# cyberfabric/cyberfabric-core

Measured on NVIDIA H100. Metric: prompt_bytes_per_sec_bpe_encode, higher is better.
Workload: dtype u32

## Files before the change

cyberfabric-core_b200/csrc/bpe_kernels.cuh:

```cuda
#pragma once
#include <stdint.h>

#include "pretok.cuh"
#include "pretok_fsm.h"
#include "pretok_sync.cuh"
#include "specials.h"
#include "tables.h"
#include "tma.cuh"

namespace cfbpe {

#ifdef CUSIM_EMULATOR
#define CFBPE_DYN_SMEM(name) uint32_t* const name = reinterpret_cast<uint32_t*>(cusim::dyn_smem())
#else
#define CFBPE_DYN_SMEM(name) extern __shared__ __align__(16) uint32_t name[]
#endif

constexpr uint32_t kMaxVocabs = 8;
#ifdef CUSIM_EMULATOR
inline unsigned long long* dbg_counters() { static unsigned long long c[16]; return c; }
#define CFBPE_DBG_COUNT(i) (++dbg_counters()[i])
#else
#define CFBPE_DBG_COUNT(i) ((void)0)
#endif
// ... 283 lines not shown
                                const uint64_t w0 = w << 5;
                                uint32_t m = pat_bits << off;
                                if (e < w0 + 32u) m &= (1u << static_cast<uint32_t>(e - w0)) - 1u;
                                if (m) atomicOr(&piece_bits[w], m);
                                off = off % md + adv; if (off >= md) off -= md;
                            }
                        }
                    }
                    state = S_D1 + static_cast<uint32_t>((d - 1u + (e - pos)) % md);
                    pos = e; prevx = X_N; nlet = 0; npun = 0;
                }
            }
#if defined(CFBPE_TILE_CLOCK) && !defined(CUSIM_EMULATOR)
            rs_bulk += clock64() - rs_b0;
#endif
        }
    }
    if (!kFix) {
        or_bits(piece_bits, cs >> 5, static_cast<uint32_t>(mine));
        or_bits(piece_bits, (cs >> 5) + 1, static_cast<uint32_t>(mine >> 32));
    }
    if (bad) atomicOr(&status->bad_utf8, 1u);
}

__global__ void __launch_bounds__(256)
pretok_split_kernel(BatchView b, VocabSet vs, UcTables uc, uint32_t* __restrict__ piece_bits, DeviceStatus* status, SplitFix* fix_list, uint32_t fix_cap) {
    __shared__ uint16_t s_fsm[kNumPatterns * kPretokTableSize];
    __shared__ uint8_t s_ascii[128];
    for (uint32_t i = threadIdx.x; i < kNumPatterns * kPretokTableSize; i += blockDim.x) s_fsm[i] = uc.fsm[i];
    if (threadIdx.x < 128) s_ascii[threadIdx.x] = uc.ascii_x[threadIdx.x];
    __syncthreads();
    const uint64_t chunk = static_cast<uint64_t>(blockIdx.x) * blockDim.x + threadIdx.x;
    const uint64_t cs = chunk * kSplitChunk;
    if (cs >= b.total_bytes) return;
    const uint64_t ce = (cs + kSplitChunk < b.total_bytes) ? cs + kSplitChunk : b.total_bytes;
    split_thread<0>(b, vs, uc, s_fsm, s_ascii, piece_bits, status, fix_list, fix_cap, cs, ce, 0, 0);
}

__global__ void __launch_bounds__(256)
pretok_fixup_kernel(BatchView b, VocabSet vs, UcTables uc, uint32_t* __restrict__ piece_bits, DeviceStatus* status, const SplitFix* fix_list, uint32_t fix_cap) {
    __shared__ uint16_t s_fsm[kNumPatterns * kPretokTableSize];
    __shared__ uint8_t s_ascii[128];
    const uint32_t n = status->fix_n < fix_cap ? status->fix_n : fix_cap;
    if (blockIdx.x * blockDim.x >= n) return;
    for (uint32_t i = threadIdx.x; i < kNumPatterns * kPretokTableSize; i += blockDim.x) s_fsm[i] = uc.fsm[i];
    if (threadIdx.x < 128) s_ascii[threadIdx.x] = uc.ascii_x[threadIdx.x];
    __syncthreads();
    for (uint32_t i = blockIdx.x * blockDim.x + threadIdx.x; i < n; i += gridDim.x * blockDim.x) {
        const SplitFix f = fix_list[i];
        split_thread<1>(b, vs, uc, s_fsm, s_ascii, piece_bits, status, nullptr, 0, 0, f.ce, f.pos, 0xFFFFFFFFu);
    }
}


constexpr uint32_t kFull = 0xFFFFFFFFu;

__device__ __forceinline__ uint32_t lanemask_lt(uint32_t lane) { return (1u << lane) - 1u; }

__device__ __forceinline__ uint64_t load_bits33(const uint32_t* __restrict__ bits, uint64_t n_words, uint64_t ws) {
    const uint64_t w = ws >> 5;
    const uint32_t sh = static_cast<uint32_t>(ws & 31);
    const uint64_t lo = bits[w];
    const uint64_t hi = (w + 1 < n_words) ? bits[w + 1] : 0;
    const uint64_t v = (lo | (hi << 32)) >> sh;
    return v & 0x1FFFFFFFFull;
}

__device__ __forceinline__ uint64_t next_set_bit(const uint32_t* __restrict__ bits, uint64_t from, uint64_t limit) {
    if (from >= limit) return limit;
    uint64_t w = from >> 5;
    uint32_t cur = bits[w] & (kFull << (from & 31));
    const uint64_t wl = (limit + 31) >> 5;
    while (!cur) {
        if (++w >= wl) return limit;
        cur = bits[w];
    }
    const uint64_t p = (w << 5) + (__ffs(cur) - 1);
    return p < limit ? p : limit;
}


constexpr uint32_t kPieceRange = 512;
constexpr uint32_t kPieceWarps = 4;

__device__ __forceinline__ void load16(const uint8_t* __restrict__ p, uint32_t& w0, uint32_t& w1, uint32_t& w2, uint32_t& w3) {
    const uintptr_t addr = reinterpret_cast<uintptr_t>(p);
    const uint32_t* q = reinterpret_cast<const uint32_t*>(addr & ~static_cast<uintptr_t>(3));
    const uint32_t sh = static_cast<uint32_t>(addr & 3) * 8;
    const uint32_t a = q[0], bq = q[1], c = q[2], d = q[3];
    if (sh == 0) { w0 = a; w1 = bq; w2 = c; w3 = d; }
    else {
        const uint32_t e = q[4];
        w0 = __funnelshift_r(a, bq, sh); w1 = __funnelshift_r(bq, c, sh); w2 = __funnelshift_r(c, d, sh); w3 = __funnelshift_r(d, e, sh);
    }
}

__device__ __forceinline__ uint32_t whole_piece_lookup(const TablesView& T, const uint8_t* __restrict__ p, uint32_t len) {
    if (len > T.max_token_len) return kNone;
    uint32_t w0, w1, w2, w3;
    load16(p, w0, w1, w2, w3);
    uint64_t k0 = static_cast<uint64_t>(w0) | (static_cast<uint64_t>(w1) << 32);
    uint32_t k1 = w2;
    if (len < 8) k0 &= (1ull << (8 * len)) - 1ull;
    if (len <= 8) k1 = 0; else if (len < 12) k1 &= (1u << (8 * (len - 8))) - 1u;
    if (len <= kShortMaxLen) return short_lookup(T, k0, k1, len);
    return long_lookup(T, long_hash(k0, k1, load_le32(p + len - 4), len), p, len);
}

__device__ __forceinline__ uint32_t merge_piece_in_lane(const TablesView& T, const uint8_t* __restrict__ text, uint64_t pos, uint32_t len,
                                                        uint32_t* sid, uint32_t* srk, uint32_t* __restrict__ tok_bits) {
    const uint8_t* __restrict__ p = text + pos;
    uint32_t w[8];
    load16(p, w[0], w[1], w[2], w[3]);
    if (len > 16) load16(p + 16, w[4], w[5], w[6], w[7]); else { w[4] = w[5] = w[6] = w[7] = 0; }
    auto byte_at = [&](uint32_t k) -> uint32_t {
        const uint32_t lo4 = (k & 4u) ? ((k & 8u) ? ((k & 16u) ? w[7] : w[3]) : ((k & 16u) ? w[5] : w[1]))
                                       : ((k & 8u) ? ((k & 16u) ? w[6] : w[2]) : ((k & 16u) ? w[4] : w[0]));
        return (lo4 >> (8u * (k & 3u))) & 0xFFu;
    };
    for (uint32_t k0 = 0; k0 < len; k0 += 4) {
        uint32_t bv[5], idv[4], rkv[4];
#pragma unroll
        for (uint32_t t = 0; t < 5; ++t) bv[t] = (k0 + t < len) ? byte_at(k0 + t) : 0u;
#pragma unroll
        for (uint32_t t = 0; t < 4; ++t) {
            idv[t] = (k0 + t < len) ? T.byte2id[bv[t]] : 0u;
            rkv[t] = (k0 + t + 1 < len) ? T.bytepair[(bv[t] << 8) | bv[t + 1]] : kNone;
        }
#pragma unroll
        for (uint32_t t = 0; t < 4; ++t) if (k0 + t < len) { sid[(k0 + t) * 32] = idv[t]; srk[(k0 + t) * 32] = rkv[t] == kNone ? kNone : ((rkv[t] << 5) | (k0 + t)); }
    }
    uint32_t alive = (len >= 32) ? kFull : ((1u << len) - 1u);
    for (;;) {
        uint32_t bkey = kNone;
        for (uint32_t bits = alive; bits; bits &= bits - 1) {
            const uint32_t k = static_cast<uint32_t>(__ffs(bits)) - 1u;
            const uint32_t r = srk[k * 32];
            bkey = r < bkey ? r : bkey;
        }
        if (bkey == kNone) break;
        const uint32_t best = bkey >> 5, bi = bkey & 31u;
        const uint32_t above = alive & ~((2u << bi) - 1u);
        const uint32_t nb = static_cast<uint32_t>(__ffs(above)) - 1u;
        alive &= ~(1u << nb);
        sid[bi * 32] = best;
        const uint32_t above2 = alive & ~((2u << bi) - 1u);
        const uint32_t below = alive & ((1u << bi) - 1u);
        const bool wr = above2 != 0, wl = below != 0;
        const uint32_t nn = wr ? static_cast<uint32_t>(__ffs(above2)) - 1u : 0u;
        const uint32_t pv = wl ? 31u - static_cast<uint32_t>(__clz(below)) : 0u;
        uint32_t nr, nl;
        pair_lookup2(T, best, wr ? sid[nn * 32] : 0u, wr, wl ? sid[pv * 32] : 0u, best, wl, nr, nl);
        srk[bi * 32] = nr == kNone ? kNone : ((nr << 5) | bi);
        if (wl) srk[pv * 32] = nl == kNone ? kNone : ((nl << 5) | pv);
    }
    const uint64_t mask = static_cast<uint64_t>(alive) << (pos & 31);
    atomicOr(&tok_bits[pos >> 5], static_cast<uint32_t>(mask));
    if (mask >> 32) atomicOr(&tok_bits[(pos >> 5) + 1], static_cast<uint32_t>(mask >> 32));
    return alive;
}

__device__ __forceinline__ uint32_t kth_set_bit(uint32_t mask, uint32_t k) {
    for (uint32_t i = 0; i < k; ++i) mask &= mask - 1;
    return __ffs(mask) - 1;
}

constexpr uint32_t kPieceMulti = 0x80000000u;
constexpr uint32_t kPieceLong = 0xFFFFFFFEu;
constexpr uint32_t kPieceTileBytes = kPieceWarps * kPieceRange;
static_assert(kPieceTileBytes == 64 * 32, "K3 derives a word's piece tile as word >> 6");
struct DenseIds {
    uint32_t* by_piece;
    uint32_t* extras;
    uint32_t extras_cap;
    uint32_t* tile_pieces;
    uint64_t* piece_base;
};

__global__ void __launch_bounds__(kPieceWarps * 32)
long_scan_kernel(BatchView b, const uint32_t* __restrict__ piece_bits, LongPiece* __restrict__ long_list, uint32_t long_cap,
                 DeviceStatus* status, uint32_t* __restrict__ tile_pieces) {
    const uint32_t lane = threadIdx.x & 31, wic = threadIdx.x >> 5;
    const uint64_t warp = static_cast<uint64_t>(blockIdx.x) * kPieceWarps + wic;
    const uint64_t r0 = warp * kPieceRange;
    const uint64_t r1 = (r0 + kPieceRange < b.total_bytes) ? r0 + kPieceRange : b.total_bytes;
    const bool multi = b.vocab_ids != nullptr;
    const uint64_t base = r0 + 16ull * lane;
    const uint32_t my = (base < b.total_bytes) ? ((piece_bits[base >> 5] >> (16u * (lane & 1u))) & 0xFFFFu) : 0u;
    uint32_t v = my ? (16u * lane + static_cast<uint32_t>(__ffs(my)) - 1u) : 0xFFFFu;
#pragma unroll
    for (uint32_t d = 1; d < 32; d <<= 1) { const uint32_t o = __shfl_down_sync(kFull, v, d); if (lane + d < 32 && o < v) v = o; }
    uint32_t nf_rel = __shfl_down_sync(kFull, v, 1);
    if (lane == 31) nf_rel = 0xFFFFu;
    const bool any_open = __any_sync(kFull, my != 0 && nf_rel == 0xFFFFu);
    uint64_t beyond = b.total_bytes;
    if (any_open) beyond = next_set_bit(piece_bits, r1, b.total_bytes);
    const uint64_t nf = (nf_rel == 0xFFFFu) ? beyond : r0 + nf_rel;
    __shared__ uint32_t s_n[2], s_at[2], s_pieces;
    __shared__ unsigned long long s_bytes;
    if (threadIdx.x < 2) s_n[threadIdx.x] = 0;
    if (threadIdx.x == 0) { s_bytes = 0; s_pieces = 0; }
    __syncthreads();
    const uint32_t np = __reduce_add_sync(kFull, static_cast<uint32_t>(__popc(my)));
    if (lane == 0 && np) atomicAdd(&s_pieces, np);
    bool is_long = false, big = false;
    uint32_t k = 0, pv = 0;
    uint64_t pos = 0;
    if (my && r0 < b.total_bytes) {
        pos = base + (31u - static_cast<uint32_t>(__clz(my)));
        if (nf - pos > 32) {
            is_long = true;
            big = (nf - pos) > kBigPiece;
            pv = multi ? b.vocab_ids[find_prompt(b.offsets, b.n_prompts, pos)] : 0u;
            k = atomicAdd(&s_n[big ? 1 : 0], 1u);
            atomicAdd(&s_bytes, static_cast<unsigned long long>(nf - pos));
        }
    }
    __syncthreads();
    if (threadIdx.x < 2 && s_n[threadIdx.x]) s_at[threadIdx.x] = atomicAdd(threadIdx.x ? &status->n_big : &status->n_long, s_n[threadIdx.x]);
    if (threadIdx.x == 2 && s_bytes) atomicAdd(&status->long_bytes, s_bytes);
    if (threadIdx.x == 3) tile_pieces[blockIdx.x] = s_pieces;
    __syncthreads();
    if (is_long) {
        const uint32_t idx = s_at[big ? 1 : 0] + k;
        if (idx < long_cap) { LongPiece lp; lp.start = pos; lp.end = nf; lp.vocab = pv; lp.pad = 0; long_list[big ? long_cap - 1 - idx : idx] = lp; }
        else atomicOr(&status->long_overflow, 1u);
    }
}

constexpr uint32_t kLookupWarps = 4;
static_assert(kLookupWarps == kPieceWarps, "K2a's CTA is the 2 KiB tile K2s counted");
__global__ void __launch_bounds__(kLookupWarps * 32)
bpe_lookup_kernel(BatchView b, VocabSet vs, const uint32_t* __restrict__ piece_bits, DenseIds dn, MissLists ml, DeviceStatus* status) {
    __shared__ uint16_t s_pos[kLookupWarps][kPieceRange + 2];
    __shared__ uint64_t s_miss0[kLookupWarps * kPieceRange / 13 + 8];
    __shared__ uint64_t s_miss1[kLookupWarps * kPieceRange / 7 + 8];
    __shared__ uint64_t s_miss2[kLookupWarps * kPieceRange / 2 + 8];
    __shared__ uint32_t s_cnt[3], s_base[3], s_nw[kLookupWarps];
    const uint32_t lane = threadIdx.x & 31, wic = threadIdx.x >> 5;
    if (threadIdx.x < 3) s_cnt[threadIdx.x] = 0;
    const uint64_t warp = static_cast<uint64_t>(blockIdx.x) * kLookupWarps + wic;
    const uint64_t r0 = warp * kPieceRange;
    const uint8_t* __restrict__ text = b.bytes;
    const bool multi = b.vocab_ids != nullptr;
    const bool in_range = r0 < b.total_bytes;
    const uint64_t r1 = (r0 + kPieceRange < b.total_bytes) ? r0 + kPieceRange : b.total_bytes;
    uint32_t n_w = 0;
    if (in_range) {
        const uint64_t base = r0 + 16ull * lane;
        const uint32_t my = (base < b.total_bytes) ? ((piece_bits[base >> 5] >> (16u * (lane & 1u))) & 0xFFFFu) : 0u;
        const uint32_t cnt = __popc(my);
        uint32_t incl = cnt;
#pragma unroll
        for (uint32_t d = 1; d < 32; d <<= 1) { const uint32_t o = __shfl_up_sync(kFull, incl, d); if (lane >= d) incl += o; }
        n_w = __shfl_sync(kFull, incl, 31);
        uint32_t slot = incl - cnt;
        for (uint32_t bits = my; bits; bits &= bits - 1) s_pos[wic][slot++] = static_cast<uint16_t>(16u * lane + static_cast<uint32_t>(__ffs(bits)) - 1u);
    }
    if (lane == 0) s_nw[wic] = n_w;
    __syncthreads();
    if (in_range) {
        uint64_t rank0 = dn.piece_base[blockIdx.x];
        for (uint32_t w = 0; w < wic; ++w) rank0 += s_nw[w];
        uint64_t beyond = b.total_bytes;
        if (n_w) beyond = next_set_bit(piece_bits, r1, b.total_bytes);
        TablesView T = vs.v[0];
        uint32_t vid = 0;
        for (uint32_t i = lane; i < n_w; i += 32) {
            const uint32_t off = s_pos[wic][i];
            const uint64_t pos = r0 + off;
            const uint64_t end = (i + 1 < n_w) ? r0 + s_pos[wic][i + 1] : beyond;
            if (end - pos > 32) { dn.by_piece[rank0 + i] = kPieceLong; continue; }
            const uint32_t len = static_cast<uint32_t>(end - pos);
            if (multi) {
                const uint32_t pv = b.vocab_ids[find_prompt(b.offsets, b.n_prompts, pos)];
                if (pv != vid) { vid = pv; T = vs.v[vid]; }
            }
            const uint32_t tok = (len == 1) ? T.byte2id[text[pos]] : whole_piece_lookup(T, text + pos, len);
            if (tok != kNone) {
                dn.by_piece[rank0 + i] = tok;
            } else {
                const uint32_t c = len >= 13 ? 0u : (len >= 7 ? 1u : 2u);
                const uint32_t k = atomicAdd(&s_cnt[c], 1u);
                (c == 0 ? s_miss0 : (c == 1 ? s_miss1 : s_miss2))[k] = pos | ((rank0 + i) << 32);
            }
        }
    }
    __syncthreads();
    if (threadIdx.x < 3) {
        const uint32_t n = s_cnt[threadIdx.x];
        uint32_t g = n ? atomicAdd(&status->miss_n[threadIdx.x], n) : 0u;
        if (n && g + n > ml.cap[threadIdx.x]) { atomicOr(&status->miss_overflow, 1u); g = 0xFFFFFFFFu; }
        s_base[threadIdx.x] = g;
    }
    __syncthreads();
#pragma unroll
    for (uint32_t c = 0; c < 3; ++c) {
        const uint32_t n = s_cnt[c], g = s_base[c];
        if (g == 0xFFFFFFFFu) continue;
        const uint64_t* src = c == 0 ? s_miss0 : (c == 1 ? s_miss1 : s_miss2);
        for (uint32_t i = threadIdx.x; i < n; i += blockDim.x) ml.list[c][g + i] = src[i];
    }
}

__global__ void __launch_bounds__(kPieceWarps * 32)
bpe_merge_kernel(BatchView b, VocabSet vs, const uint32_t* __restrict__ piece_bits, DenseIds dn,
                 uint32_t* __restrict__ tok_bits, MissLists ml, DeviceStatus* status) {
    __shared__ uint32_t s_id[kPieceWarps][32][32];
    __shared__ uint32_t s_rk[kPieceWarps][32][32];
    const uint32_t lane = threadIdx.x & 31, wic = threadIdx.x >> 5;
    const uint8_t* __restrict__ text = b.bytes;
    const bool multi = b.vocab_ids != nullptr;
    uint32_t* sid = &s_id[wic][0][lane];
    uint32_t* srk = &s_rk[wic][0][lane];
    if (status->miss_overflow) return;
    TablesView T = vs.v[0];
    uint32_t vid = 0;
#pragma unroll 1
    for (uint32_t c = 0; c < 3; ++c) {
        const uint32_t n = status->miss_n[c];
        const uint64_t* __restrict__ list = ml.list[c];
        for (;;) {
            uint32_t t0 = 0;
            if (lane == 0) t0 = atomicAdd(&status->miss_next[c], 32u);
            t0 = __shfl_sync(kFull, t0, 0);
            if (t0 >= n) break;
            const uint32_t i = t0 + lane;
            uint32_t alive = 0, rank = 0;
            if (i < n) {
                const uint64_t e = list[i];
                const uint64_t pos = e & 0xFFFFFFFFull;
                rank = static_cast<uint32_t>(e >> 32);
                const uint64_t end = next_set_bit(piece_bits, pos + 1, b.total_bytes);
                if (multi) {
                    const uint32_t pv = b.vocab_ids[find_prompt(b.offsets, b.n_prompts, pos)];
                    if (pv != vid) { vid = pv; T = vs.v[vid]; }
                }
                alive = merge_piece_in_lane(T, text, pos, static_cast<uint32_t>(end - pos), sid, srk, tok_bits);
            }
            const uint32_t cnt = __popc(alive);
            uint32_t incl = cnt;
#pragma unroll
            for (uint32_t d = 1; d < 32; d <<= 1) { const uint32_t o = __shfl_up_sync(kFull, incl, d); if (lane >= d) incl += o; }
            const uint32_t total = __shfl_sync(kFull, incl, 31);
            uint32_t base = 0;
            if (lane == 0 && total) base = atomicAdd(&status->extra_n, total);
            base = __shfl_sync(kFull, base, 0);
            if (cnt) {
                uint32_t slot = base + incl - cnt;
                if (slot + cnt <= dn.extras_cap) {
                    dn.by_piece[rank] = kPieceMulti | slot;
                    for (uint32_t bits = alive; bits; bits &= bits - 1) dn.extras[slot++] = sid[(static_cast<uint32_t>(__ffs(bits)) - 1u) * 32];
                } else atomicOr(&status->miss_overflow, 1u);
            }
            __syncwarp();
        }
    }
}

struct LongScratch {
    uint32_t* rank;
    uint32_t* aux0;
    uint32_t* aux1;
};

__device__ __forceinline__ uint32_t warp_min_u32(uint32_t v) {
#pragma unroll
    for (uint32_t d = 16; d; d >>= 1) { const uint32_t o = __shfl_xor_sync(kFull, v, d); v = o < v ? o : v; }
    return v;
}

__device__ __forceinline__ bool select_chunk(uint32_t r, uint32_t rmin, uint32_t lane, uint32_t& carry, uint32_t& sel_ballot) {
    const bool cand = (r == rmin);
    const uint32_t C = __ballot_sync(kFull, cand);
    const uint32_t z = ~C & lanemask_lt(lane);
    const uint32_t s = z ? (32u - __clz(z)) : 0u;
    const uint32_t cnt = lane - s + (s == 0 ? carry : 0u);
    const bool sel = cand && !(cnt & 1u);
    sel_ballot = __ballot_sync(kFull, sel);
    const uint32_t nz = ~C;
    carry = nz ? static_cast<uint32_t>(__clz(nz)) : (carry + 32u);
    return sel;
}

// ... 1030 lines not shown
```

cyberfabric-core_b200/csrc/pipeline.cuh:

```cuda
#pragma once
#include "../../include/cfbpe.h"
#include "bpe_kernels.cuh"

namespace cfbpe {

struct Workspace {
    uint32_t* piece_bits;
    uint32_t* tok_bits;
    uint32_t* ids_by_pos;
    LongScratch lscratch;
    LongPiece* long_list;
    uint32_t long_cap;
    uint32_t* tile_counts;
    uint64_t* tile_base;
    DeviceStatus* status;
    MissLists miss;
    SplitFix* fix_list;
    uint32_t fix_cap;
    DenseIds dense;
    uint32_t* pstart_bits;
    uint32_t* block_prompt;
};

enum WsKind : uint32_t {
// ... 32 lines not shown

inline uint64_t miss_list_words(uint64_t max_bytes, uint32_t c, uint32_t max_chunks) {
    return workspace_alloc(max_bytes, max_chunks).n[kWsMiss0 + c];
}

template <typename F>
inline void for_each_ws_buffer(Workspace& w, F&& f) {
    f(w.piece_bits, kWsFlagWords); f(w.tok_bits, kWsFlagWords); f(w.pstart_bits, kWsFlagWords);
    f(w.ids_by_pos, kWsPerByte); f(w.lscratch.rank, kWsPerByte); f(w.lscratch.aux0, kWsPerByte); f(w.lscratch.aux1, kWsPerByte);
    f(w.dense.by_piece, kWsPerByte); f(w.dense.extras, kWsPerByte);
    f(w.long_list, kWsLongList);
    f(w.tile_counts, kWsScanTiles); f(w.tile_base, kWsScanTiles);
    f(w.miss.list[0], kWsMiss0); f(w.miss.list[1], kWsMiss1); f(w.miss.list[2], kWsMiss2);
    f(w.fix_list, kWsFixList);
    f(w.dense.tile_pieces, kWsPieceTiles); f(w.dense.piece_base, kWsPieceTiles);
    f(w.block_prompt, kWsBlockPrompt);
}

inline void set_workspace_caps(Workspace& w, const WsSizes& s) {
    w.long_cap = static_cast<uint32_t>(s.n[kWsLongList]);
    w.fix_cap = static_cast<uint32_t>(s.n[kWsFixList]);
    w.dense.extras_cap = static_cast<uint32_t>(s.n[kWsPerByte]);
    for (uint32_t c = 0; c < 3; ++c) w.miss.cap[c] = static_cast<uint32_t>(s.n[kWsMiss0 + c]);
}

inline Workspace slice_workspace(const Workspace& all, uint64_t o0, uint64_t len, uint32_t k) {
    Workspace w = all;
    for_each_ws_buffer(w, [&](auto*& p, WsKind kind) { p += o0 / kWsRules[kind].unit + static_cast<uint64_t>(kWsRules[kind].per_k) * k; });
    set_workspace_caps(w, workspace_extent(len));
    return w;
}

inline uint64_t sub_batch_bytes_at(uint64_t o0, uint32_t k) { return ((o0 + 15) & ~15ull) + 16ull * k; }
inline uint64_t lane_bytes_alloc(uint64_t max_bytes, uint32_t max_chunks) { return max_bytes + 256 + 16ull * (max_chunks + 1); }
inline uint64_t sub_batch_offsets_at(uint32_t p0, uint32_t k) { return static_cast<uint64_t>(p0) + k; }
inline uint64_t lane_offsets_alloc(uint64_t max_prompts, uint32_t max_chunks) { return max_prompts + 1 + max_chunks; }

struct StatusError { int code; const char* msg; };
inline StatusError status_error(const DeviceStatus& st) {
    if (st.long_overflow || st.miss_overflow) return {CFBPE_EIO, "internal: long-piece list overflow"};
    if (st.bad_vocab) return {CFBPE_ENOENT, "a prompt names a vocabulary that is not loaded"};
    if (st.bad_utf8) return {CFBPE_EILSEQ, "a prompt holds malformed UTF-8"};
    return {CFBPE_OK, nullptr};
}

inline const char* truncate_args_error(const uint32_t* budgets, uint32_t mode, const uint32_t* cut, const uint32_t* kept) {
    if (mode != CFBPE_TRUNCATE_HEAD && mode != CFBPE_TRUNCATE_TAIL) return "mode is not a CFBPE_TRUNCATE_* value";
    if (!budgets || !cut || !kept) return "budgets, out_cut and out_kept are required";
    return nullptr;
}

inline const char* chunk_args_error(uint32_t chunk_tokens, uint32_t overlap_tokens, const uint32_t* spans, const uint64_t* chunk_offsets) {
    if (chunk_tokens == 0) return "chunk_tokens must be at least 1";
    if (overlap_tokens >= chunk_tokens) return "overlap_tokens must be less than chunk_tokens";
    if (!spans || !chunk_offsets) return "out_spans and out_chunk_offsets are required";
    return nullptr;
}

#ifndef CFBPE_LONG_CTAS
#define CFBPE_LONG_CTAS 8
#endif
constexpr uint32_t kLongCtasPerSm = CFBPE_LONG_CTAS;
#ifndef CFBPE_LIST_CTAS
#define CFBPE_LIST_CTAS 3
#endif
constexpr uint32_t kListCtasPerSm = CFBPE_LIST_CTAS;

enum KernelIdx { K_SPLIT = 0, K_ENCODE = 1, K_LONG = 2, K_COUNT = 3, K_SCAN = 4, K_EMIT = 5, K_LIST = 6, K_LONGSCAN = 7, K_MERGE = 8 };

inline uint64_t n_flag_words(uint64_t total_bytes) { return (total_bytes + 31) >> 5; }
inline uint32_t n_scan_tiles(uint64_t total_bytes) {
    return static_cast<uint32_t>((n_flag_words(total_bytes) + kScanTileWords - 1) / kScanTileWords);
}

template <typename Stream, typename Prof>
inline void enqueue_split(const BatchView& b, const VocabSet& vs, const UcTables& uc, const Workspace& w, Stream stream, Prof* prof,
                          uint32_t sm_count) {
    const uint64_t nw = n_flag_words(b.total_bytes);
    CFBPE_ZERO(w.status, sizeof(DeviceStatus), stream);
    if (!b.total_bytes) return;
    CFBPE_ZERO(w.piece_bits, (nw + 2) * sizeof(uint32_t), stream);
    CFBPE_ZERO(w.tok_bits, (nw + 2) * sizeof(uint32_t), stream);
    CFBPE_MARK(prof, K_SPLIT, stream, true);
#ifdef CFBPE_SPLIT_LEGACY
    const uint64_t n_chunks = (b.total_bytes + kSplitChunk - 1) / kSplitChunk;
    CFBPE_LAUNCH(pretok_split_kernel, static_cast<unsigned>((n_chunks + 255) / 256), 256, stream, b, vs, uc, w.piece_bits, w.status, w.fix_list, w.fix_cap);
#else
    CFBPE_ZERO(w.pstart_bits, (nw + 2) * sizeof(uint32_t), stream);
    CFBPE_LAUNCH(prompt_map_kernel, static_cast<unsigned>((static_cast<uint64_t>(b.n_prompts) + 1 + 255) / 256), 256, stream, b, vs, w.pstart_bits, w.block_prompt, w.status);
    {
        const uint64_t n_blocks16 = (b.total_bytes + 15) / 16;
        const uint32_t n_tiles = static_cast<uint32_t>((n_blocks16 + kSplitWarpOwned - 1) / kSplitWarpOwned);
        const uint32_t n_tabs = b.vocab_ids ? kNumPatterns : 1u;
        const uint32_t cap = sm_count * CFBPE_SPLIT_CTAS;
        const uint32_t n_ctas = (n_tiles + kSplitCta / 32 - 1) / (kSplitCta / 32);
        CFBPE_LAUNCH_SMEM(pretok_split16_kernel, n_ctas < cap ? n_ctas : cap, kSplitCta, n_tabs * kProdTableBytes, stream,
                          b, vs, uc, w.pstart_bits, w.block_prompt, w.piece_bits, w.status, w.fix_list, w.fix_cap, n_tabs, n_tiles);
    }
#endif
    CFBPE_LAUNCH(pretok_fixup_kernel, 2 * sm_count, 256, stream, b, vs, uc, w.piece_bits, w.status, w.fix_list, w.fix_cap);
    CFBPE_MARK(prof, K_SPLIT, stream, false);
    const uint64_t n_warps = (b.total_bytes + kPieceRange - 1) / kPieceRange;
    CFBPE_MARK(prof, K_LONGSCAN, stream, true);
    CFBPE_LAUNCH(long_scan_kernel, static_cast<unsigned>((n_warps + kPieceWarps - 1) / kPieceWarps), kPieceWarps * 32, stream,
                 b, w.piece_bits, w.long_list, w.long_cap, w.status, w.dense.tile_pieces);
    CFBPE_MARK(prof, K_LONGSCAN, stream, false);
}

template <typename Stream, typename Prof>
inline void enqueue_short(const BatchView& b, const VocabSet& vs, const Workspace& w, uint32_t long_grid, Stream stream, Prof* prof) {
    if (!b.total_bytes) return;
    const uint64_t n_warps = (b.total_bytes + kPieceRange - 1) / kPieceRange;
    CFBPE_MARK(prof, K_ENCODE, stream, true);
    const uint32_t n_tiles2k = static_cast<uint32_t>((n_warps + kLookupWarps - 1) / kLookupWarps);
    CFBPE_LAUNCH(tile_scan_kernel, 1u, 1024, stream, w.dense.tile_pieces, n_tiles2k, w.dense.piece_base, static_cast<DeviceStatus*>(nullptr),
                 static_cast<const uint64_t*>(nullptr));
    CFBPE_LAUNCH(bpe_lookup_kernel, n_tiles2k, kLookupWarps * 32, stream, b, vs, w.piece_bits, w.dense, w.miss, w.status);
    CFBPE_MARK(prof, K_ENCODE, stream, false);
    CFBPE_MARK(prof, K_MERGE, stream, true);
    CFBPE_LAUNCH(bpe_merge_kernel, long_grid + long_grid / 2, kPieceWarps * 32, stream,
                 b, vs, w.piece_bits, w.dense, w.tok_bits, w.miss, w.status);
    CFBPE_MARK(prof, K_MERGE, stream, false);
}

template <typename Stream, typename Prof>
inline void enqueue_long(const BatchView& b, const VocabSet& vs, const Workspace& w, uint32_t long_grid, Stream stream, Prof* prof) {
    if (!b.total_bytes) return;
    CFBPE_MARK(prof, K_LONG, stream, true);
    CFBPE_LAUNCH(bpe_long_kernel, (long_grid / 4) * kLongCtasPerSm, kLongWarps * 32, stream, b, vs, w.long_list, w.status, w.long_cap, w.ids_by_pos, w.lscratch, w.tok_bits);
    CFBPE_MARK(prof, K_LONG, stream, false);
}
template <typename Stream, typename Prof>
inline void enqueue_list(const BatchView& b, const VocabSet& vs, const Workspace& w, uint32_t long_grid, Stream stream, Prof* prof) {
    if (!b.total_bytes) return;
#ifndef CFBPE_NO_DEFER
    CFBPE_MARK(prof, K_LIST, stream, true);
    CFBPE_LAUNCH_SMEM(bpe_list_kernel, (long_grid / 4) * kListCtasPerSm, kListWarps * 32, kListSmemBytes, stream, b, vs, w.long_list, w.status, w.long_cap, w.ids_by_pos, w.lscratch, w.tok_bits);
    CFBPE_MARK(prof, K_LIST, stream, false);
#endif
}

template <typename Stream, typename Prof>
inline void enqueue_count(const BatchView& b, const Workspace& w, Stream stream, Prof* prof) {
    if (!b.total_bytes) return;
    CFBPE_MARK(prof, K_COUNT, stream, true);
    CFBPE_LAUNCH(flag_count_kernel, n_scan_tiles(b.total_bytes), 256, stream, w.tok_bits, w.piece_bits, n_flag_words(b.total_bytes), w.tile_counts);
    CFBPE_MARK(prof, K_COUNT, stream, false);
}
template <typename Stream, typename Prof>
inline void enqueue_scan(const BatchView& b, const Workspace& w, Stream stream, Prof* prof, const uint64_t* token_base) {
    if (b.total_bytes) {
        CFBPE_MARK(prof, K_SCAN, stream, true);
        CFBPE_LAUNCH(tile_scan_kernel, 1u, 1024, stream, w.tile_counts, n_scan_tiles(b.total_bytes), w.tile_base, w.status, token_base);
        CFBPE_MARK(prof, K_SCAN, stream, false);
    } else {
        CFBPE_LAUNCH(tile_scan_kernel, 1u, 32, stream, w.tile_counts, 0u, w.tile_base, w.status, token_base);
    }
}
constexpr uint32_t kChunkEmitCtas = 1024;
template <typename Stream, typename Prof>
inline void enqueue_emit(const BatchView& b, const Workspace& w, uint32_t* out_ids, uint64_t out_cap, uint64_t* out_offsets,
                         uint32_t* out_counts, Stream stream, Prof* prof, uint32_t* out_starts = nullptr, const VocabSet* vs = nullptr,
                         const TruncateView* trunc = nullptr, const ChunkView* chunk = nullptr) {
    CFBPE_MARK(prof, K_EMIT, stream, true);
    if (b.total_bytes && out_ids) {
        CFBPE_LAUNCH(emit_compact_kernel, n_scan_tiles(b.total_bytes), 256, stream, w.tok_bits, w.piece_bits, n_flag_words(b.total_bytes), w.tile_base,
                     w.dense, w.ids_by_pos, out_ids, out_cap);
    }
    CFBPE_LAUNCH(prompt_offsets_kernel, static_cast<unsigned>((static_cast<uint64_t>(b.n_prompts) + 1 + 7) / 8), 256, stream,
                 b, w.tok_bits, w.tile_base, out_offsets, out_counts, w.status);
    CFBPE_MARK(prof, K_EMIT, stream, false);
    if (b.total_bytes && out_ids && out_starts) {
        const uint32_t n_tiles = static_cast<uint32_t>((b.total_bytes + kStartsTile - 1) / kStartsTile);
        CFBPE_LAUNCH(starts_len_kernel, n_tiles, 256, stream, b, *vs, out_ids, out_offsets, out_cap, w.status, out_starts, w.dense.tile_pieces);
        CFBPE_LAUNCH(tile_scan_kernel, 1u, 1024, stream, w.dense.tile_pieces, n_tiles, w.dense.piece_base, static_cast<DeviceStatus*>(nullptr),
                     static_cast<const uint64_t*>(nullptr));
        CFBPE_LAUNCH(starts_emit_kernel, n_tiles, 256, stream, b, out_offsets, out_cap, w.status, w.dense.piece_base, out_starts);
    }
    if (out_ids && trunc && b.n_prompts) {
        CFBPE_LAUNCH(truncate_kernel, static_cast<unsigned>((static_cast<uint64_t>(b.n_prompts) + 7) / 8), 256, stream,
                     b, *vs, out_ids, out_offsets, *trunc);
        if (b.total_bytes > kTruncChunkBytes) {
            const uint64_t n_chunks = (b.total_bytes + kTruncChunkBytes - 1) / kTruncChunkBytes;
            CFBPE_LAUNCH(truncate_long_kernel, static_cast<unsigned>((n_chunks + 7) / 8), 256, stream, b, *vs, out_ids, out_offsets, *trunc);
        }
    }
    if (out_ids && out_starts && chunk) {
        CFBPE_LAUNCH(chunk_scan_kernel, 1u, 1024, stream, b, out_offsets, *chunk, w.status);
        if (b.total_bytes) {
            const uint64_t ctas = (b.total_bytes + 255) / 256;
            CFBPE_LAUNCH(chunk_emit_kernel, static_cast<unsigned>(ctas < kChunkEmitCtas ? ctas : kChunkEmitCtas), 256, stream,
                         b, out_offsets, static_cast<const uint32_t*>(out_starts), *chunk, static_cast<const DeviceStatus*>(w.status));
        }
    }
}
template <typename Stream, typename Prof>
inline void enqueue_back(const BatchView& b, const Workspace& w, uint32_t* out_ids, uint64_t out_cap, uint64_t* out_offsets,
                         uint32_t* out_counts, Stream stream, Prof* prof, const uint64_t* token_base, uint32_t* out_starts = nullptr,
                         const VocabSet* vs = nullptr, const TruncateView* trunc = nullptr, const ChunkView* chunk = nullptr) {
    enqueue_count(b, w, stream, prof);
// ... 23 lines not shown
```

cyberfabric-core_b200/csrc/pretok_lanes.cuh:

```cuda
#pragma once
#include "pretok_ctx.h"

namespace cfbpe {

constexpr uint32_t kSplitCta = 256;
constexpr uint32_t kPromptBlockShift = 9;
constexpr uint32_t kNoRow = 0xFFFFu;

__device__ __forceinline__ uint32_t bit_at(const uint32_t* __restrict__ bits, uint64_t pos) { return (bits[pos >> 5] >> (pos & 31)) & 1u; }

__device__ __forceinline__ uint32_t prompt_at(const BatchView& b, const uint32_t* __restrict__ block_prompt, uint64_t pos) {
    uint32_t p = block_prompt[pos >> kPromptBlockShift];
    while (b.offsets[p + 1] <= pos) ++p;
    return p;
}

__global__ void __launch_bounds__(256)
prompt_map_kernel(BatchView b, VocabSet vs, uint32_t* __restrict__ pstart_bits, uint32_t* __restrict__ block_prompt, DeviceStatus* status) {
    const uint64_t i = static_cast<uint64_t>(blockIdx.x) * blockDim.x + threadIdx.x;
    if (i > b.n_prompts) return;
    if (i == b.n_prompts) { atomicOr(&pstart_bits[b.total_bytes >> 5], 1u << (b.total_bytes & 31)); return; }
    const uint64_t s = b.offsets[i], e = b.offsets[i + 1];
    if (b.vocab_ids) {
        const uint32_t v = b.vocab_ids[i];
        if (v >= kMaxVocabs || !((vs.loaded_mask >> v) & 1u)) atomicOr(&status->bad_vocab, 1u);
    }
    if (e <= s) return;
    atomicOr(&pstart_bits[s >> 5], 1u << (s & 31));
    for (uint64_t blk = (s + (1u << kPromptBlockShift) - 1) >> kPromptBlockShift; (blk << kPromptBlockShift) < e; ++blk)
        block_prompt[blk] = static_cast<uint32_t>(i);
}

__device__ __noinline__ uint4 classify_non_ascii(const uint8_t* __restrict__ s, uint64_t base, uint64_t total, const uint32_t* __restrict__ pstart_bits,
                                                 const UcTables uc, uint4 raw, uint4 cwv, uint32_t P, DeviceStatus* status) {
    uint32_t bad = 0;
    uint32_t need = 0;
    if ((raw.x & 0xC0u) == 0x80u && !(P & 1u)) {
        for (uint32_t j = 1; j <= 3 && j <= base; ++j) {
            if (j > 1 && bit_at(pstart_bits, base - j + 1)) break;
            const uint32_t c = s[base - j];
            if ((c & 0xC0u) == 0x80u) continue;
            if (c >= 0xC0u) { const uint32_t len = c < 0xE0u ? 2u : (c < 0xF0u ? 3u : 4u); if (len > j) need = len - j; }
            break;
        }
    }
    const uint64_t lo = raw.x | (static_cast<uint64_t>(raw.y) << 32), hi = raw.z | (static_cast<uint64_t>(raw.w) << 32);
    const uint64_t ext = load_u32_any(s + base + 16);
    uint64_t clo = cwv.x | (static_cast<uint64_t>(cwv.y) << 32), chi = cwv.z | (static_cast<uint64_t>(cwv.w) << 32);
    const uint32_t n = total - base < 16 ? static_cast<uint32_t>(total - base) : 16u;
    const uint32_t valid = n >= 16 ? 0xFFFFu : ((1u << n) - 1u);
    auto byte_mask = [](uint32_t w0, uint32_t w1, uint32_t w2, uint32_t w3, uint32_t v) -> uint32_t {
        uint32_t m = 0;
        const uint32_t ws[4] = {w0, w1, w2, w3};
#pragma unroll
        for (uint32_t j = 0; j < 4; ++j) {
            const uint32_t nz = (((ws[j] ^ (v * 0x01010101u)) & 0x7F7F7F7Fu) + 0x7F7F7F7Fu) | (ws[j] ^ (v * 0x01010101u));
            m |= (((((~nz) & 0x80808080u) >> 7) * 0x01020408u) >> 24 & 15u) << (4u * j);
        }
        return m;
    };
    const uint32_t conts = byte_mask(cwv.x, cwv.y, cwv.z, cwv.w, X_CONT) & valid;
    uint32_t leads = byte_mask(cwv.x, cwv.y, cwv.z, cwv.w, X_LEAD) & valid;
    uint32_t expected = (1u << need) - 1u;
    while (leads) {
        const uint32_t k = static_cast<uint32_t>(__ffs(leads)) - 1u;
        leads &= leads - 1u;
        const uint32_t w = k < 8 ? static_cast<uint32_t>(k ? ((lo >> (8u * k)) | (hi << (64u - 8u * k))) : lo)
                                 : static_cast<uint32_t>(k > 8 ? ((hi >> (8u * (k - 8u))) | (ext << (64u - 8u * (k - 8u)))) : hi);
        const uint32_t b0 = w & 0xFFu, b1 = (w >> 8) & 0xFFu, b2 = (w >> 16) & 0xFFu, b3 = w >> 24;
        uint32_t len, cp;
        bool ok;
        if (b0 >= 0xC2u && b0 <= 0xDFu) { len = 2; cp = ((b0 & 0x1Fu) << 6) | (b1 & 0x3Fu); ok = (b1 & 0xC0u) == 0x80u; }
        else if (b0 >= 0xE0u && b0 <= 0xEFu) {
            len = 3; cp = ((b0 & 0x0Fu) << 12) | ((b1 & 0x3Fu) << 6) | (b2 & 0x3Fu);
            ok = (b1 & 0xC0u) == 0x80u && (b2 & 0xC0u) == 0x80u && cp >= 0x800u && !(cp >= 0xD800u && cp <= 0xDFFFu);
        } else if (b0 >= 0xF0u && b0 <= 0xF4u) {
            len = 4; cp = ((b0 & 0x07u) << 18) | ((b1 & 0x3Fu) << 12) | ((b2 & 0x3Fu) << 6) | (b3 & 0x3Fu);
            ok = (b1 & 0xC0u) == 0x80u && (b2 & 0xC0u) == 0x80u && (b3 & 0xC0u) == 0x80u && cp >= 0x10000u && cp <= 0x10FFFFu;
        } else { len = 1; cp = 0; ok = false; }
        ok = ok && k + len <= n + (total - base > 16 ? 4u : 0u) && !((P >> (k + 1)) & ((1u << (len - 1u)) - 1u));
        uint32_t cb;
        if (!ok) { bad = 1; len = 1; cb = X_OTHER; }
        else cb = uc_class(uc, cp) | ((len - 1u) << 4);
        expected |= ((1u << (len - 1u)) - 1u) << (k + 1u);
        if (k < 8) clo = (clo & ~(0xFFull << (8u * k))) | (static_cast<uint64_t>(cb) << (8u * k));
        else chi = (chi & ~(0xFFull << (8u * (k - 8u)))) | (static_cast<uint64_t>(cb) << (8u * (k - 8u)));
    }
    if ((conts & ~expected) != 0u) bad = 1;
    if (bad) atomicOr(&status->bad_utf8, 1u);
// ... 395 lines not shown
```

Before: 35.98 billion.

## Stage warp text in shared memory and batch hash-table probes in lookup kernel

The lookup kernel now copies each warp's 512-byte text range (plus slack) into shared memory with coalesced loads and builds keys from there instead of doing unaligned global loads per piece. Pieces are compacted into short and long lists, and short-table probes are issued in batches so several global loads are in flight per lane. Per-piece binary-search prompt lookup is replaced by a block_prompt map and a warp-level check for prompt boundaries, which needs prompt_map_kernel to run on every path. Miss lists are packed to 32-bit entries in shared memory to reduce footprint, and the kernel gets a min-blocks-per-SM launch bound, at the cost of more shared memory and register pressure.

```diff
diff --git a/cyberfabric-core_b200/csrc/bpe_kernels.cuh b/cyberfabric-core_b200/csrc/bpe_kernels.cuh
--- a/cyberfabric-core_b200/csrc/bpe_kernels.cuh
+++ b/cyberfabric-core_b200/csrc/bpe_kernels.cuh
@@ -389,6 +389,7 @@
 
 constexpr uint32_t kPieceRange = 512;
 constexpr uint32_t kPieceWarps = 4;
+constexpr uint32_t kPromptBlockShift = 9;
 
 __device__ __forceinline__ void load16(const uint8_t* __restrict__ p, uint32_t& w0, uint32_t& w1, uint32_t& w2, uint32_t& w3) {
     const uintptr_t addr = reinterpret_cast<uintptr_t>(p);
@@ -402,16 +403,36 @@
     }
 }
 
-__device__ __forceinline__ uint32_t whole_piece_lookup(const TablesView& T, const uint8_t* __restrict__ p, uint32_t len) {
-    if (len > T.max_token_len) return kNone;
-    uint32_t w0, w1, w2, w3;
-    load16(p, w0, w1, w2, w3);
-    uint64_t k0 = static_cast<uint64_t>(w0) | (static_cast<uint64_t>(w1) << 32);
-    uint32_t k1 = w2;
+__device__ __forceinline__ uint32_t staged_u32(const uint32_t* st, uint32_t q) {
+    return __funnelshift_r(st[q >> 2], st[(q >> 2) + 1], (q & 3u) * 8u);
+}
+__device__ __forceinline__ void staged_key(const uint32_t* st, uint32_t q, uint32_t len, uint64_t& k0, uint32_t& k1) {
+    const uint32_t w = q >> 2, sh = (q & 3u) * 8u;
+    const uint32_t a = st[w], bq = st[w + 1], c = st[w + 2], d = st[w + 3];
+    k0 = static_cast<uint64_t>(__funnelshift_r(a, bq, sh)) | (static_cast<uint64_t>(__funnelshift_r(bq, c, sh)) << 32);
+    k1 = __funnelshift_r(c, d, sh);
     if (len < 8) k0 &= (1ull << (8 * len)) - 1ull;
     if (len <= 8) k1 = 0; else if (len < 12) k1 &= (1u << (8 * (len - 8))) - 1u;
-    if (len <= kShortMaxLen) return short_lookup(T, k0, k1, len);
-    return long_lookup(T, long_hash(k0, k1, load_le32(p + len - 4), len), p, len);
+}
+__device__ __forceinline__ uint32_t staged_long_lookup(const TablesView& T, uint64_t hash, const uint32_t* st, uint32_t q, uint32_t len) {
+    uint32_t h = static_cast<uint32_t>(hash >> 17) & T.long_mask;
+    for (;;) {
+        const uint4 s = __ldg(reinterpret_cast<const uint4*>(T.lng + h));
+        if (s.z == kMetaEmpty) return kNone;
+        if ((static_cast<uint64_t>(s.x) | (static_cast<uint64_t>(s.y) << 32)) == hash && (s.z >> 24) == len) {
+            const uint32_t id = s.z & 0x00FFFFFFu;
+            const uint8_t* t = T.blob + s.w;
+            const uint32_t n0 = T.tokoff[id], n1 = T.tokoff[id + 1];
+            uint32_t diff = 0;
+#pragma unroll
+            for (uint32_t i = 0; i < 32; i += 4) {
+                const uint32_t o = i + 4 <= len ? i : len - 4;
+                diff |= load_u32_any(t + o) ^ staged_u32(st, q + o);
+            }
+            if (diff == 0 && n1 - n0 == len) return id;
+        }
+        h = (h + 1) & T.long_mask;
+    }
 }
 
 __device__ __forceinline__ uint32_t merge_piece_in_lane(const TablesView& T, const uint8_t* __restrict__ text, uint64_t pos, uint32_t len,
@@ -537,12 +558,31 @@
 
 constexpr uint32_t kLookupWarps = 4;
 static_assert(kLookupWarps == kPieceWarps, "K2a's CTA is the 2 KiB tile K2s counted");
-__global__ void __launch_bounds__(kLookupWarps * 32)
-bpe_lookup_kernel(BatchView b, VocabSet vs, const uint32_t* __restrict__ piece_bits, DenseIds dn, MissLists ml, DeviceStatus* status) {
+static_assert((1u << kPromptBlockShift) == kPieceRange, "K2a takes its first prompt from block_prompt[warp]");
+#ifndef CFBPE_LOOKUP_BATCH
+#define CFBPE_LOOKUP_BATCH 4
+#endif
+constexpr uint32_t kLookupBatch = CFBPE_LOOKUP_BATCH;
+constexpr uint32_t kLookupCtasPerSm = 10;
+constexpr uint32_t kStageBytes = kPieceRange + 32;
+constexpr uint32_t kStageWords = (3 + kStageBytes + 3 + 15) / 16 * 4;
+constexpr uint32_t kStageLoads = (kStageWords + 31) / 32;
+constexpr uint32_t kNoEntry = 0xFFFFFFFFu;
+__device__ __forceinline__ uint32_t lookup_entry(uint32_t i, uint32_t off, uint32_t len, uint32_t vid) { return i | off << 9 | len << 18 | vid << 24; }
+__device__ __forceinline__ uint32_t entry_index(uint32_t e) { return e & 511u; }
+__device__ __forceinline__ uint32_t entry_off(uint32_t e) { return (e >> 9) & 511u; }
+__device__ __forceinline__ uint32_t entry_len(uint32_t e) { return (e >> 18) & 63u; }
+
+__global__ void __launch_bounds__(kLookupWarps * 32, kLookupCtasPerSm)
+bpe_lookup_kernel(BatchView b, VocabSet vs, const uint32_t* __restrict__ piece_bits, const uint32_t* __restrict__ pstart_bits,
+                  const uint32_t* __restrict__ block_prompt, DenseIds dn, MissLists ml, DeviceStatus* status) {
+    __shared__ __align__(16) uint32_t s_text[kLookupWarps][kStageWords];
     __shared__ uint16_t s_pos[kLookupWarps][kPieceRange + 2];
-    __shared__ uint64_t s_miss0[kLookupWarps * kPieceRange / 13 + 8];
-    __shared__ uint64_t s_miss1[kLookupWarps * kPieceRange / 7 + 8];
-    __shared__ uint64_t s_miss2[kLookupWarps * kPieceRange / 2 + 8];
+    __shared__ uint32_t s_mid[kLookupWarps][kPieceRange / 2];
+    __shared__ uint32_t s_lng[kLookupWarps][kPieceRange / 13 + 1];
+    __shared__ uint32_t s_miss0[kLookupWarps * kPieceRange / 13 + 8];
+    __shared__ uint32_t s_miss1[kLookupWarps * kPieceRange / 7 + 8];
+    __shared__ uint32_t s_miss2[kLookupWarps * kPieceRange / 2 + 8];
     __shared__ uint32_t s_cnt[3], s_base[3], s_nw[kLookupWarps];
     const uint32_t lane = threadIdx.x & 31, wic = threadIdx.x >> 5;
     if (threadIdx.x < 3) s_cnt[threadIdx.x] = 0;
@@ -552,10 +592,30 @@
     const bool multi = b.vocab_ids != nullptr;
     const bool in_range = r0 < b.total_bytes;
     const uint64_t r1 = (r0 + kPieceRange < b.total_bytes) ? r0 + kPieceRange : b.total_bytes;
-    uint32_t n_w = 0;
+    const uint64_t tile_base = dn.piece_base[blockIdx.x];
+    uint32_t* st = s_text[wic];
+    uint32_t sh = 0, n_w = 0, nxt = 0, p0 = 0, vid_w = 0;
+    bool vsplit = false;
     if (in_range) {
+        const uintptr_t a0 = reinterpret_cast<uintptr_t>(text + r0);
+        sh = static_cast<uint32_t>(a0 & 3u);
+        const uint32_t* g = reinterpret_cast<const uint32_t*>(text + r0 - sh);
+        const uint64_t lim = (r0 + kStageBytes < b.total_bytes) ? r0 + kStageBytes : b.total_bytes;
+        const uint32_t n_words = (sh + static_cast<uint32_t>(lim - r0) + 3u) >> 2;
+        uint32_t tw[kStageLoads];
+#pragma unroll
+        for (uint32_t k = 0; k < kStageLoads; ++k) { const uint32_t j = lane + 32u * k; tw[k] = j < n_words ? g[j] : 0u; }
         const uint64_t base = r0 + 16ull * lane;
         const uint32_t my = (base < b.total_bytes) ? ((piece_bits[base >> 5] >> (16u * (lane & 1u))) & 0xFFFFu) : 0u;
+        if (r1 < b.total_bytes) nxt = piece_bits[r1 >> 5];
+        if (multi) {
+            p0 = block_prompt[warp];
+            uint32_t ps = (base < b.total_bytes) ? ((pstart_bits[base >> 5] >> (16u * (lane & 1u))) & 0xFFFFu) : 0u;
+            if (base < b.total_bytes && base + 16 > b.total_bytes) ps &= (1u << static_cast<uint32_t>(b.total_bytes - base)) - 1u;
+            if (lane == 0) ps &= ~1u;
+            vsplit = __any_sync(kFull, ps != 0);
+            vid_w = b.vocab_ids[p0];
+        }
         const uint32_t cnt = __popc(my);
         uint32_t incl = cnt;
 #pragma unroll
@@ -563,34 +623,117 @@
         n_w = __shfl_sync(kFull, incl, 31);
         uint32_t slot = incl - cnt;
         for (uint32_t bits = my; bits; bits &= bits - 1) s_pos[wic][slot++] = static_cast<uint16_t>(16u * lane + static_cast<uint32_t>(__ffs(bits)) - 1u);
+#pragma unroll
+        for (uint32_t k = 0; k < kStageLoads; ++k) { const uint32_t j = lane + 32u * k; if (j < kStageWords) st[j] = tw[k]; }
     }
     if (lane == 0) s_nw[wic] = n_w;
     __syncthreads();
-    if (in_range) {
-        uint64_t rank0 = dn.piece_base[blockIdx.x];
-        for (uint32_t w = 0; w < wic; ++w) rank0 += s_nw[w];
+    if (in_range && n_w) {
+        uint32_t rank_t = 0;
+        for (uint32_t w = 0; w < wic; ++w) rank_t += s_nw[w];
+        const uint64_t rank0 = tile_base + rank_t;
         uint64_t beyond = b.total_bytes;
-        if (n_w) beyond = next_set_bit(piece_bits, r1, b.total_bytes);
-        TablesView T = vs.v[0];
-        uint32_t vid = 0;
-        for (uint32_t i = lane; i < n_w; i += 32) {
-            const uint32_t off = s_pos[wic][i];
-            const uint64_t pos = r0 + off;
-            const uint64_t end = (i + 1 < n_w) ? r0 + s_pos[wic][i + 1] : beyond;
-            if (end - pos > 32) { dn.by_piece[rank0 + i] = kPieceLong; continue; }
-            const uint32_t len = static_cast<uint32_t>(end - pos);
-            if (multi) {
-                const uint32_t pv = b.vocab_ids[find_prompt(b.offsets, b.n_prompts, pos)];
-                if (pv != vid) { vid = pv; T = vs.v[vid]; }
-            }
-            const uint32_t tok = (len == 1) ? T.byte2id[text[pos]] : whole_piece_lookup(T, text + pos, len);
+        if (nxt) beyond = r1 + static_cast<uint32_t>(__ffs(nxt)) - 1u;
+        else if (r1 < b.total_bytes) beyond = next_set_bit(piece_bits, r1 + 32, b.total_bytes);
+        if (beyond > b.total_bytes) beyond = b.total_bytes;
+        auto finish = [&](uint32_t e, uint32_t tok) {
+            const uint32_t i = entry_index(e), len = entry_len(e);
             if (tok != kNone) {
                 dn.by_piece[rank0 + i] = tok;
             } else {
+                CFBPE_DBG_COUNT(11);
                 const uint32_t c = len >= 13 ? 0u : (len >= 7 ? 1u : 2u);
                 const uint32_t k = atomicAdd(&s_cnt[c], 1u);
-                (c == 0 ? s_miss0 : (c == 1 ? s_miss1 : s_miss2))[k] = pos | ((rank0 + i) << 32);
-            }
+                (c == 0 ? s_miss0 : (c == 1 ? s_miss1 : s_miss2))[k] = (wic * kPieceRange + entry_off(e)) | ((rank_t + i) << 16);
+            }
+        };
+        const uint32_t lt = (1u << lane) - 1u;
+        uint32_t n_mid = 0, n_lng = 0;
+        for (uint32_t i0 = 0; i0 < n_w; i0 += 32) {
+            const uint32_t i = i0 + lane;
+            uint32_t e = 0;
+            bool mid = false, lng = false;
+            if (i < n_w) {
+                const uint32_t off = s_pos[wic][i];
+                const uint64_t end = (i + 1 < n_w) ? r0 + s_pos[wic][i + 1] : beyond;
+                if (end - (r0 + off) > 32) {
+                    dn.by_piece[rank0 + i] = kPieceLong;
+                } else {
+                    const uint32_t len = static_cast<uint32_t>(end - (r0 + off));
+                    uint32_t vid = vid_w;
+                    if (vsplit) {
+                        uint32_t p = p0;
+                        while (b.offsets[p + 1] <= r0 + off) ++p;
+                        vid = b.vocab_ids[p];
+                    }
+                    vid = vid < kMaxVocabs ? vid : 0u;
+                    if (len == 1) {
+                        const uint32_t q = sh + off;
+                        dn.by_piece[rank0 + i] = __ldg(&vs.v[vid].byte2id[(st[q >> 2] >> ((q & 3u) * 8u)) & 0xFFu]);
+                    } else {
+                        e = lookup_entry(i, off, len, vid);
+                        mid = len <= kShortMaxLen;
+                        lng = !mid;
+                    }
+                }
+            }
+            const uint32_t bm = __ballot_sync(kFull, mid), bl = __ballot_sync(kFull, lng);
+            if (mid) s_mid[wic][n_mid + __popc(bm & lt)] = e;
+            if (lng) s_lng[wic][n_lng + __popc(bl & lt)] = e;
+            n_mid += __popc(bm);
+            n_lng += __popc(bl);
+        }
+        __syncwarp();
+        for (uint32_t j0 = 0; j0 < n_mid; j0 += 32 * kLookupBatch) {
+            uint32_t e[kLookupBatch], h[kLookupBatch];
+            uint4 sl[kLookupBatch];
+#pragma unroll
+            for (uint32_t k = 0; k < kLookupBatch; ++k) {
+                const uint32_t j = j0 + 32 * k + lane;
+                e[k] = j < n_mid ? s_mid[wic][j] : kNoEntry;
+                h[k] = 0;
+                sl[k] = make_uint4(0, 0, 0, kMetaEmpty);
+                if (e[k] != kNoEntry) {
+                    const TablesView& T = vs.v[e[k] >> 24];
+                    const uint32_t len = entry_len(e[k]);
+                    if (len <= T.max_token_len) {
+                        uint64_t k0; uint32_t k1;
+                        staged_key(st, sh + entry_off(e[k]), len, k0, k1);
+                        h[k] = short_hash(k0, k1, len) & T.short_mask;
+                        sl[k] = __ldg(reinterpret_cast<const uint4*>(T.shrt + h[k]));
+                    }
+                }
+            }
+#pragma unroll
+            for (uint32_t k = 0; k < kLookupBatch; ++k) {
+                if (e[k] == kNoEntry) continue;
+                const TablesView& T = vs.v[e[k] >> 24];
+                const uint32_t len = entry_len(e[k]);
+                uint64_t k0; uint32_t k1;
+                staged_key(st, sh + entry_off(e[k]), len, k0, k1);
+                uint32_t tok = kNone;
+                uint4 s = sl[k];
+                while (s.w != kMetaEmpty) {
+                    if ((static_cast<uint64_t>(s.x) | (static_cast<uint64_t>(s.y) << 32)) == k0 && s.z == k1 && (s.w >> 24) == len) {
+                        tok = s.w & 0x00FFFFFFu;
+                        break;
+                    }
+                    h[k] = (h[k] + 1) & T.short_mask;
+                    s = __ldg(reinterpret_cast<const uint4*>(T.shrt + h[k]));
+                }
+                finish(e[k], tok);
+            }
+        }
+        for (uint32_t j = lane; j < n_lng; j += 32) {
+            const uint32_t e = s_lng[wic][j], len = entry_len(e), q = sh + entry_off(e);
+            const TablesView& T = vs.v[e >> 24];
+            uint32_t tok = kNone;
+            if (len <= T.max_token_len) {
+                uint64_t k0; uint32_t k1;
+                staged_key(st, q, len, k0, k1);
+                tok = staged_long_lookup(T, long_hash(k0, k1, staged_u32(st, q + len - 4), len), st, q, len);
+            }
+            finish(e, tok);
         }
     }
     __syncthreads();
@@ -601,12 +744,16 @@
         s_base[threadIdx.x] = g;
     }
     __syncthreads();
+    const uint64_t tile_r0 = static_cast<uint64_t>(blockIdx.x) * kPieceTileBytes;
 #pragma unroll
     for (uint32_t c = 0; c < 3; ++c) {
         const uint32_t n = s_cnt[c], g = s_base[c];
         if (g == 0xFFFFFFFFu) continue;
-        const uint64_t* src = c == 0 ? s_miss0 : (c == 1 ? s_miss1 : s_miss2);
-        for (uint32_t i = threadIdx.x; i < n; i += blockDim.x) ml.list[c][g + i] = src[i];
+        const uint32_t* src = c == 0 ? s_miss0 : (c == 1 ? s_miss1 : s_miss2);
+        for (uint32_t i = threadIdx.x; i < n; i += blockDim.x) {
+            const uint32_t v = src[i];
+            ml.list[c][g + i] = (tile_r0 + (v & 0xFFFFu)) | ((tile_base + (v >> 16)) << 32);
+        }
     }
 }
 
diff --git a/cyberfabric-core_b200/csrc/pipeline.cuh b/cyberfabric-core_b200/csrc/pipeline.cuh
--- a/cyberfabric-core_b200/csrc/pipeline.cuh
+++ b/cyberfabric-core_b200/csrc/pipeline.cuh
@@ -138,12 +138,12 @@
     CFBPE_ZERO(w.piece_bits, (nw + 2) * sizeof(uint32_t), stream);
     CFBPE_ZERO(w.tok_bits, (nw + 2) * sizeof(uint32_t), stream);
     CFBPE_MARK(prof, K_SPLIT, stream, true);
+    CFBPE_ZERO(w.pstart_bits, (nw + 2) * sizeof(uint32_t), stream);
+    CFBPE_LAUNCH(prompt_map_kernel, static_cast<unsigned>((static_cast<uint64_t>(b.n_prompts) + 1 + 255) / 256), 256, stream, b, vs, w.pstart_bits, w.block_prompt, w.status);
 #ifdef CFBPE_SPLIT_LEGACY
     const uint64_t n_chunks = (b.total_bytes + kSplitChunk - 1) / kSplitChunk;
     CFBPE_LAUNCH(pretok_split_kernel, static_cast<unsigned>((n_chunks + 255) / 256), 256, stream, b, vs, uc, w.piece_bits, w.status, w.fix_list, w.fix_cap);
 #else
-    CFBPE_ZERO(w.pstart_bits, (nw + 2) * sizeof(uint32_t), stream);
-    CFBPE_LAUNCH(prompt_map_kernel, static_cast<unsigned>((static_cast<uint64_t>(b.n_prompts) + 1 + 255) / 256), 256, stream, b, vs, w.pstart_bits, w.block_prompt, w.status);
     {
         const uint64_t n_blocks16 = (b.total_bytes + 15) / 16;
         const uint32_t n_tiles = static_cast<uint32_t>((n_blocks16 + kSplitWarpOwned - 1) / kSplitWarpOwned);
@@ -171,7 +171,8 @@
     const uint32_t n_tiles2k = static_cast<uint32_t>((n_warps + kLookupWarps - 1) / kLookupWarps);
     CFBPE_LAUNCH(tile_scan_kernel, 1u, 1024, stream, w.dense.tile_pieces, n_tiles2k, w.dense.piece_base, static_cast<DeviceStatus*>(nullptr),
                  static_cast<const uint64_t*>(nullptr));
-    CFBPE_LAUNCH(bpe_lookup_kernel, n_tiles2k, kLookupWarps * 32, stream, b, vs, w.piece_bits, w.dense, w.miss, w.status);
+    CFBPE_LAUNCH(bpe_lookup_kernel, n_tiles2k, kLookupWarps * 32, stream, b, vs, w.piece_bits, w.pstart_bits, w.block_prompt, w.dense, w.miss,
+                 w.status);
     CFBPE_MARK(prof, K_ENCODE, stream, false);
     CFBPE_MARK(prof, K_MERGE, stream, true);
     CFBPE_LAUNCH(bpe_merge_kernel, long_grid + long_grid / 2, kPieceWarps * 32, stream,
diff --git a/cyberfabric-core_b200/csrc/pretok_lanes.cuh b/cyberfabric-core_b200/csrc/pretok_lanes.cuh
--- a/cyberfabric-core_b200/csrc/pretok_lanes.cuh
+++ b/cyberfabric-core_b200/csrc/pretok_lanes.cuh
@@ -4,7 +4,6 @@
 namespace cfbpe {
 
 constexpr uint32_t kSplitCta = 256;
-constexpr uint32_t kPromptBlockShift = 9;
 constexpr uint32_t kNoRow = 0xFFFFu;
 
 __device__ __forceinline__ uint32_t bit_at(const uint32_t* __restrict__ bits, uint64_t pos) { return (bits[pos >> 5] >> (pos & 31)) & 1u; }
```

Result: faster. 37.12 billion (median of 6 runs) (+3.2%).
